# TRI-ML/sdflabel

Hardware: AMD Instinct MI355X
Metric: rendered rays/sec (fwd+bwd) (higher is better)
Workload: dtype f32; 1 GPU; BASELINE configs[1]: one 256x256 crop(s) per GPU, DeepSDF 8x512 on a 40^3 grid, fwd+bwd to yaw/trans/latent, decoder re-evaluated every step; crops_per_gpu=1, rays_per_crop=65536, grid_points=64000, surfels=2751, front_facing=763, parallelism=crop-parallel x1

## Files before the change

sdflabel_amd/csrc/mlp.hip:

```cpp
#include "mlp_kernel.h"
#include <cmath>
#include <stdlib.h>
#include <string.h>
#include <vector>


#define SDFR_DEVICE_CHECK(d, what)                                                                                                          \
    do {                                                                                                                                    \
        int cur_ = -1;                                                                                                                      \
        SDFR_HIP_CHECK(hipGetDevice(&cur_));                                                                                                \
        SDFR_REQUIRE(cur_ == (d)->device, "%s: the decoder's weights live on device %d but the current device (the launch stream's) is %d: " \
                     "create one decoder handle per device", what, (d)->device, cur_);                                                      \
    } while (0)

extern "C" int sdfr_decoder_create(sdfr_decoder** out, int n_lin, const int* in_dim, const int* out_dim,
                                   const int* inj_n, const int* inj_off, const float* const* h_W,
                                   const float* const* h_b, const float* const* h_ln_w, const float* const* h_ln_b, int n_inputs,
                                   int use_tanh, int device) {
    SDFR_REQUIRE(out && in_dim && out_dim && inj_n && inj_off && h_W && h_b, "sdfr_decoder_create: NULL argument");
    SDFR_REQUIRE(n_lin >= 2 && n_lin <= SDFR_MAX_LAYERS, "sdfr_decoder_create: n_lin=%d outside [2,%d]", n_lin, SDFR_MAX_LAYERS);
    SDFR_REQUIRE(out_dim[n_lin - 1] == 1, "sdfr_decoder_create: last layer must have out_dim 1 (got %d)", out_dim[n_lin - 1]);
    SDFR_REQUIRE(in_dim[0] == n_inputs && inj_n[0] == 0, "sdfr_decoder_create: layer 0 must consume exactly the input row");
    int width = 0;
    for (int l = 0; l < n_lin; ++l) {
// ... 36 lines not shown
    for (int l = 0; l < n_lin - 1; ++l) {
        const MlpLayer& L = P.L[l];
        const float* W = h_W[l];
        for (int r = 0; r < L.out_dim; ++r)
            for (int k = 0; k < L.in_dim; ++k) {
                const float w = W[(size_t)r * L.in_dim + k];
                Wf[((size_t)L.off_f + (size_t)(k / 4) * HP + r) * 4 + (k % 4)] = w;
                const _Float16 wh = (_Float16)w;
                const int prev_out = l > 0 ? P.L[l - 1].out_dim : 0;
                const int kh = (kinj && l > 0 && L.inj_n > 0 && k >= prev_out) ? HP + L.inj_off + (k - prev_out) : k;
                Wh[((size_t)L.off_h + (size_t)(kh / 8) * HP + r) * 8 + (kh % 8)] = wh;
                const size_t es = ((size_t)L.off_s + ((size_t)(k / 8) * HP + r) * 2) * 8 + (k % 8);
                Ws[es] = wh;
                Ws[es + 8] = (_Float16)((w - (float)wh) * 2048.f);
                Wb[((size_t)L.off_b + (size_t)(r / 4) * HP + k) * 4 + (r % 4)] = w;
                Wbh[((size_t)L.off_bh + (size_t)(r / 8) * HP + k) * 8 + (r % 8)] = wh;
            }
        for (int r = 0; r < L.out_dim; ++r) bias[(size_t)l * HP + r] = h_b[l][r];
    }
    std::vector<float> Wk;
    bool finite = true;
    if (HP == 512 && !d->has_ln) {
        Wk.assign((size_t)off_f * 4, 0.f);
        for (int l = 0; l < n_lin - 1; ++l) {
            const MlpLayer& L = P.L[l];
            for (int r = 0; r < L.out_dim; ++r)
                for (int k = 0; k < L.in_dim; ++k) {
                    const float w = h_W[l][(size_t)r * L.in_dim + k];
                    finite = finite && std::isfinite(w);
                    Wk[(size_t)L.off_f * 4 + (size_t)k * HP + sdfr_wk_row(r)] = w;
                }
        }
    }
    for (int k = 0; k < in_dim[n_lin - 1]; ++k) wl[k] = h_W[n_lin - 1][k];
    P.b_last = h_b[n_lin - 1][0];

    SDFR_HIP_CHECK(hipMalloc(&d->d_Wf, Wf.size() * sizeof(float)));
    SDFR_HIP_CHECK(hipMalloc(&d->d_Wb, Wb.size() * sizeof(float)));
    if (d->has_ln) {
        std::vector<float> lg((size_t)(n_lin - 1) * HP, 0.f), lb((size_t)(n_lin - 1) * HP, 0.f);
        for (int l = 0; l < n_lin - 1; ++l)
            if (P.L[l].ln)
                for (int r = 0; r < P.L[l].out_dim; ++r) { lg[(size_t)l * HP + r] = h_ln_w[l][r]; lb[(size_t)l * HP + r] = h_ln_b[l][r]; }
        SDFR_HIP_CHECK(hipMalloc(&d->d_lng, lg.size() * sizeof(float)));
        SDFR_HIP_CHECK(hipMalloc(&d->d_lnb, lb.size() * sizeof(float)));
        SDFR_HIP_CHECK(hipMemcpy(d->d_lng, lg.data(), lg.size() * sizeof(float), hipMemcpyHostToDevice));
        SDFR_HIP_CHECK(hipMemcpy(d->d_lnb, lb.data(), lb.size() * sizeof(float), hipMemcpyHostToDevice));
        P.ln_gamma = d->d_lng; P.ln_beta = d->d_lnb;
    }
    SDFR_HIP_CHECK(hipMalloc(&d->d_Wh, Wh.size() * sizeof(_Float16)));
    SDFR_HIP_CHECK(hipMemcpy(d->d_Wh, Wh.data(), Wh.size() * sizeof(_Float16), hipMemcpyHostToDevice));
    SDFR_HIP_CHECK(hipMalloc(&d->d_Wbh, Wbh.size() * sizeof(_Float16)));
    SDFR_HIP_CHECK(hipMemcpy(d->d_Wbh, Wbh.data(), Wbh.size() * sizeof(_Float16), hipMemcpyHostToDevice));
    SDFR_HIP_CHECK(hipMalloc(&d->d_Ws, Ws.size() * sizeof(_Float16)));
    SDFR_HIP_CHECK(hipMemcpy(d->d_Ws, Ws.data(), Ws.size() * sizeof(_Float16), hipMemcpyHostToDevice));
    SDFR_HIP_CHECK(hipMalloc(&d->d_bias, bias.size() * sizeof(float)));
    SDFR_HIP_CHECK(hipMalloc(&d->d_wlast, wl.size() * sizeof(float)));
    SDFR_HIP_CHECK(hipMemcpy(d->d_Wf, Wf.data(), Wf.size() * sizeof(float), hipMemcpyHostToDevice));
    SDFR_HIP_CHECK(hipMemcpy(d->d_Wb, Wb.data(), Wb.size() * sizeof(float), hipMemcpyHostToDevice));
    SDFR_HIP_CHECK(hipMemcpy(d->d_bias, bias.data(), bias.size() * sizeof(float), hipMemcpyHostToDevice));
    SDFR_HIP_CHECK(hipMemcpy(d->d_wlast, wl.data(), wl.size() * sizeof(float), hipMemcpyHostToDevice));
    if (!Wk.empty()) {
        SDFR_HIP_CHECK(hipMalloc(&d->d_Wk, Wk.size() * sizeof(float)));
        SDFR_HIP_CHECK(hipMemcpy(d->d_Wk, Wk.data(), Wk.size() * sizeof(float), hipMemcpyHostToDevice));
        P.Wk = d->d_Wk;
        P.kcompact = finite ? 1 : 0;
    }
    P.Wf = d->d_Wf; P.Wb = d->d_Wb; P.Wh = d->d_Wh; P.Ws = d->d_Ws; P.Wbh = d->d_Wbh; P.bias = d->d_bias; P.w_last = d->d_wlast; P.fwd_np = 2;
    *out = d;
    return SDFR_OK;
}

static unsigned long long* g_trace = nullptr;
extern "C" int sdfr_debug_set_trace(void* device_buffer) { g_trace = (unsigned long long*)device_buffer; return SDFR_OK; }

extern "C" int sdfr_decoder_destroy(sdfr_decoder* d) {
    if (!d) return SDFR_OK;
    void* bufs[] = {d->d_Wf, d->d_Wb, d->d_Wk, d->d_Wh, d->d_Ws, d->d_Wbh, d->d_bias, d->d_wlast, d->d_lng, d->d_lnb, d->ln_ws};
    for (void* b : bufs) (void)hipFree(b);
    delete d;
    return SDFR_OK;
}

extern "C" int64_t sdfr_decoder_macs(const sdfr_decoder* d) { return d ? d->macs : 0; }

static void mask_geometry(int HP, int* ft, int* nt) {
    if (HP == 128) { *ft = 1; *nt = 256; }
    else if (HP == 256) { *ft = 2; *nt = 256; }
    else { *ft = 2; *nt = 512; }
}

extern "C" int64_t sdfr_decoder_mask_words(const sdfr_decoder* d, int64_t n) {
    if (!d || n <= 0) return 0;
    int ft, nt;
    mask_geometry(d->HP, &ft, &nt);
    return ((n + 127) / 128) * 2 * (int64_t)(d->n_lin - 1) * ft * nt;
}

extern "C" int sdfr_mlp_forward(const sdfr_decoder* d, const float* inputs, int64_t n, float* sdf, uint32_t* mask_ws, void* stream) {
    SDFR_REQUIRE(d && inputs && sdf, "sdfr_mlp_forward: NULL argument");
    SDFR_DEVICE_CHECK(d, "sdfr_mlp_forward");
    SDFR_REQUIRE(n >= 0 && n < (int64_t)1 << 31, "sdfr_mlp_forward: n=%lld out of range", (long long)n);
    if (n == 0) return SDFR_OK;
    MlpParams P = d->proto;
    P.inputs = inputs; P.n = n; P.sdf = sdf; P.maskbuf = mask_ws; P.trace = g_trace;
    const int grid = sdfr_cdiv(n, 64);
    if (d->has_ln) sdfr_launch_ln(P, d->HP, false, grid, 1, (hipStream_t)stream);
    else if (d->HP == 512) sdfr_launch_fwd_f32_512(P, n, mask_ws != nullptr, (hipStream_t)stream);
    else sdfr_launch_small(P, d->HP, mask_ws ? 1 : 0, grid, 1, (hipStream_t)stream);
    SDFR_LAUNCH_CHECK();
    return SDFR_OK;
// ... 257 lines not shown
```

sdflabel_amd/csrc/mlp_jac.hip:

```cpp
#include "mlp_kernel.h"
#ifndef SDFR_JAC_MS
#define SDFR_JAC_MS 32
#define SDFR_JAC_FT 4
#define SDFR_JAC_NP 1
#define SDFR_JAC_NW 4
#define SDFR_JAC_PF 2
#endif
#ifndef SDFR_JAC_SMALL_FT
#define SDFR_JAC_SMALL_FT 8
#define SDFR_JAC_SMALL_NW 4
#define SDFR_JAC_SMALL_PF 4
#endif
#ifndef SDFR_JAC_SWITCH_ROWS
#define SDFR_JAC_SWITCH_ROWS 8
#endif
void sdfr_launch_jac_f32_512_recompute32(const MlpParams& P, int cap, int B, hipStream_t s) {
    hipLaunchKernelGGL((sdfr_mlp_kernel<float, 32, 4, 1, 4, 2, 2>), dim3(sdfr_cdiv(cap, 32), B), dim3(256), 0, s, P);
}

#include <stdlib.h>
static int jac_pool_crops() {
    static const int v = [] { const char* e = getenv("SDFR_JAC_POOL_CROPS"); return e ? atoi(e) : 12; }();
    return v;
}
void sdfr_launch_jac_f32_512(const MlpParams& P, int cap, int B, bool from_masks, hipStream_t s) {
    static_assert(SDFR_JAC_MS * SDFR_JAC_FT * SDFR_JAC_NW == 512 && 16 * SDFR_JAC_SMALL_FT * SDFR_JAC_SMALL_NW == 512, "padded width 512 = MS * FT * NW");
    if (!from_masks) {
        hipLaunchKernelGGL((sdfr_mlp_kernel<float, 16, 8, 1, 4, 4, 2>), dim3(sdfr_cdiv(cap, 16), B), dim3(256), 0, s, P);
    } else if (B >= jac_pool_crops() && B <= 64 && P.n_crops == B) {
        const int64_t tiles = (int64_t)sdfr_cdiv(cap, SDFR_JAC_MS * SDFR_JAC_NP) * B;
        hipLaunchKernelGGL((sdfr_mlp_kernel<float, SDFR_JAC_MS, SDFR_JAC_FT, SDFR_JAC_NP, SDFR_JAC_NW, SDFR_JAC_PF, 3, 0, false, 2>),
                           dim3((unsigned)(tiles < 512 ? tiles : 512)), dim3(64 * SDFR_JAC_NW), 0, s, P);
    } else if (B >= SDFR_JAC_SWITCH_ROWS) {
        hipLaunchKernelGGL((sdfr_mlp_kernel<float, SDFR_JAC_MS, SDFR_JAC_FT, SDFR_JAC_NP, SDFR_JAC_NW, SDFR_JAC_PF, 3>),
                           dim3(sdfr_cdiv(cap, SDFR_JAC_MS * SDFR_JAC_NP), B), dim3(64 * SDFR_JAC_NW), 0, s, P);
    } else {
        hipLaunchKernelGGL((sdfr_mlp_kernel<float, 16, SDFR_JAC_SMALL_FT, 1, SDFR_JAC_SMALL_NW, SDFR_JAC_SMALL_PF, 3>), dim3(sdfr_cdiv(cap, 16), B),
                           dim3(64 * SDFR_JAC_SMALL_NW), 0, s, P);
    }
}

void sdfr_launch_fwd_f32_512_tile16(const MlpParams& P, int64_t n, hipStream_t s) {
    hipLaunchKernelGGL((sdfr_mlp_kernel<float, 16, SDFR_JAC_SMALL_FT, 1, SDFR_JAC_SMALL_NW, SDFR_JAC_SMALL_PF, 0>), dim3(sdfr_cdiv(n, 16)),
                       dim3(64 * SDFR_JAC_SMALL_NW), 0, s, P);
}

void sdfr_launch_tail_f32_512(const MlpParams& P, int64_t n_rays, int spec_k, hipStream_t s) {
    const dim3 grid(sdfr_cdiv(n_rays, P.t_rt));
    if (spec_k > 1)
        hipLaunchKernelGGL((sdfr_mlp_kernel<float, 16, SDFR_JAC_SMALL_FT, 4, SDFR_JAC_SMALL_NW, 2, 4>), grid, dim3(64 * SDFR_JAC_SMALL_NW), 0, s, P);
    else
        hipLaunchKernelGGL((sdfr_mlp_kernel<float, 16, SDFR_JAC_SMALL_FT, 1, SDFR_JAC_SMALL_NW, SDFR_JAC_SMALL_PF, 4>), grid, dim3(64 * SDFR_JAC_SMALL_NW), 0,
                           s, P);
}
```

sdflabel_amd/csrc/mlp_kernel.h:

```cpp
#pragma once
#include "sdfr_common.h"
#include "kc_slots.h"
#include <math.h>
#include <type_traits>

typedef float f32x16 __attribute__((ext_vector_type(16)));
typedef float f32x4 __attribute__((ext_vector_type(4)));
typedef _Float16 h16;
typedef h16 h16x8 __attribute__((ext_vector_type(8)));
typedef h16 h16x4 __attribute__((ext_vector_type(4)));

struct MlpLayer {
    int in_dim, out_dim;
    int inj_n, inj_off;
    int kp_f, kp_b, kp_h;
    int off_f, off_b, off_h;
    int kp_bh, off_bh;
    int kp_s, off_s;
    int ln;
};

struct MlpParams {
    const float4* Wf;
    const float4* Wb;
    const void* Wh;
    const void* Wbh;
    const void* Ws;
    const float* Wk;
    int kcompact;
    int kinj;
    int fwd_np;
    const float* bias;
    const float* ln_gamma;
    const float* ln_beta;
    float4* ln_ws;
// ... 18 lines not shown
    int64_t skip_rows;
    const int32_t* crop_cnt;
    int64_t crop_rows;
    const int32_t* gather_idx;
    int64_t gather_rows;
    int n_crops;
    const int32_t* n_dev;
    int n_dev_lo, n_dev_hi;
    unsigned long long* trace;
    float* t_rows;
    int t_rt;
    const float* t_latn;
    const int32_t* t_pix;
    const float4* t_lam;
    int t_step0;
    int t_nlv;
    int t_lv_from[SDFR_TRACE_LEVELS], t_lv_k[SDFR_TRACE_LEVELS];
    float t_qmax;
    int32_t* t_tile_ctr;
    int t_stage;
    int32_t* t_next_cnt;
    int32_t* t_next_pix;
    float4* t_next_lam;
    const float* t_far;
    const float* t_pose;
    const float* t_Kinv;
    float* t_hit_lam;
    float* t_hit_sdf;
    int t_W, t_H, t_steps;
    const int32_t* t_wh; int t_PS;
    float t_eps, t_sigma;
    unsigned long long* t_evals;
    int32_t* t_unresolved;
};

struct sdfr_decoder {
    int device;
    int n_lin, n_inputs, use_tanh, HP;
    float4* d_Wf;
    float4* d_Wb;
    float* d_Wk;
    void* d_Wh;
    void* d_Ws;
    void* d_Wbh;
    float* d_lng;
    float* d_lnb;
    int has_ln;
    mutable float4* ln_ws;
    mutable size_t ln_ws_bytes;
    float* d_bias;
    float* d_wlast;
    int64_t macs;
    MlpParams proto;
};

__device__ __forceinline__ float f4c(const float4& v, int i) { return i == 0 ? v.x : (i == 1 ? v.y : (i == 2 ? v.z : v.w)); }

template <typename ET, int MS> struct Mma;
template <> struct Mma<float, 32> {
    typedef f32x16 acc_t; typedef float4 vec_t;
    static constexpr int KV = 4, NSTEP = 4;
    static __device__ __forceinline__ acc_t step(const vec_t& a, const vec_t& b, acc_t c, int ks) {
        return __builtin_amdgcn_mfma_f32_32x32x2f32(f4c(a, ks), f4c(b, ks), c, 0, 0, 0);
    }
};
template <> struct Mma<float, 16> {
    typedef f32x4 acc_t; typedef float4 vec_t;
    static constexpr int KV = 4, NSTEP = 4;
    static __device__ __forceinline__ acc_t step(const vec_t& a, const vec_t& b, acc_t c, int ks) {
        return __builtin_amdgcn_mfma_f32_16x16x4f32(f4c(a, ks), f4c(b, ks), c, 0, 0, 0);
    }
};
template <> struct Mma<h16, 32> {
    typedef f32x16 acc_t; typedef h16x8 vec_t;
// ... 1 lines not shown
    static __device__ __forceinline__ acc_t step(const vec_t& a, const vec_t& b, acc_t c, int) {
#ifdef SDFR_ABL_NOMFMA
        c[0] += (float)a[0] * (float)b[0];
        return c;
#else
        return __builtin_amdgcn_mfma_f32_32x32x16_f16(a, b, c, 0, 0, 0);
#endif
    }
};
template <> struct Mma<h16, 16> {
    typedef f32x4 acc_t; typedef h16x8 vec_t;
    static constexpr int KV = 8, NSTEP = 1;
    static __device__ __forceinline__ acc_t step(const vec_t& a, const vec_t& b, acc_t c, int) {
        return __builtin_amdgcn_mfma_f32_16x16x32_f16(a, b, c, 0, 0, 0);
    }
};
__device__ __forceinline__ void store4(float* dst, const float* v) { *reinterpret_cast<float4*>(dst) = make_float4(v[0], v[1], v[2], v[3]); }
__device__ __forceinline__ void store4(h16* dst, const float* v) {
    h16x4 t; t[0] = (h16)v[0]; t[1] = (h16)v[1]; t[2] = (h16)v[2]; t[3] = (h16)v[3];
    *reinterpret_cast<h16x4*>(dst) = t;
}

__device__ __forceinline__ int64_t sdfr_mask_dword(int64_t r, int l, int n_layers, int HP32, int j) {
    return (((r >> 7) * n_layers + l) * 128 + (r & 127)) * HP32 + (j >> 5);
}
__host__ __device__ __forceinline__ int sdfr_wk_row(int r) { return (r & ~63) | ((r & 31) << 1) | ((r >> 5) & 1); }
__device__ __forceinline__ int sdfr_mask_shift(int j) { return ((j >> 2) & 1) * 16 + ((j & 31) >> 3) * 4 + (j & 3); }

#ifndef SDFR_MLP_WPE
#define SDFR_MLP_WPE 1
#endif
template <typename ET, int MS, int FT, int NP, int NW, int MODE, bool LN, int XF> constexpr bool sdfr_mlp_kc2() {
    return sizeof(ET) == 4 && MS == 32 && FT == 2 && NP == 1 && NW == 8 && (MODE == 0 || MODE == 1) && !LN && (XF & ~4) == 0;
}
template <typename ET, int MS, int FT, int NP, int NW, int PF, int MODE, int PFB_ = 0, bool LN = false, int XF = 0>
__global__ __launch_bounds__(64 * NW, (sdfr_mlp_kc2<ET, MS, FT, NP, NW, MODE, LN, XF>() ? 4 : SDFR_MLP_WPE)) void sdfr_mlp_kernel(const MlpParams P) {
    typedef Mma<ET, MS> M;
    typedef typename M::acc_t acc_t;
    typedef typename M::vec_t vec_t;
    constexpr bool HALF = sizeof(ET) == 2;
    constexpr bool JAC = MODE == 2 || MODE == 3;
    constexpr bool TAIL = MODE == 4;
    constexpr bool SAVE = MODE == 1;
    constexpr bool LMASK = MODE == 2;
    constexpr bool GMASK = MODE == 3;
    constexpr bool GATHER = (XF & 1) != 0;
    constexpr bool PERSIST = (XF & 2) != 0;
    constexpr bool ORDER = (XF & 4) != 0;
    static_assert(!ORDER || (XF == 4 && (MODE == 0 || MODE == 1) && sizeof(ET) == 4 && MS == 32 && FT == 2), "ORDER: the exact-f32 grid forward alone");
    static_assert(XF == 0 || (MODE == 0 || MODE == 1) || (MODE == 3 && XF == 2), "GATHER is a forward feature; PERSIST: forward modes and the mask-fed Jacobian");
    constexpr bool JPOOL = JAC && PERSIST;
    static_assert(!SAVE || MS == 32, "mask layout assumes 32x32 forward tiles");
    static_assert(!SAVE || (FT * NP) % 2 == 0, "mask words: FT*NP*16 bits per thread and layer must fill whole words");
    static_assert(!HALF || !JAC || MODE == 3, "with half operands only the mask-fed Jacobian exists (MODE 3)");
    static_assert(!LN || (!HALF && MODE != 1 && MODE != 3 && MODE != 4), "LayerNorm decoders: float32 forward (MODE 0) and recomputing Jacobian (MODE 2)");
    static_assert(!TAIL || (NP * MS <= 64 && (NP * MS) % 16 == 0), "tail march: the tile's rows (t_rt rays x K samples) live in wave 0");
    constexpr int KV = M::KV;
    constexpr int NLG = 64 / MS;
    constexpr int RG = MS / (4 * NLG);
    constexpr int KT = KV * NLG;
    constexpr int NT = 64 * NW;
    constexpr int PT = MS * NP;
    constexpr int HP = MS * FT * NW;
    constexpr int KG = HP / KV;
    constexpr int FT32 = HP / (32 * NW);
    constexpr int MW = (FT * NP * RG * 4 + 31) / 32;
    constexpr int MASK_WORDS = LMASK ? (SDFR_MAX_LAYERS * MW * NT) : 1;
    constexpr int LN_F4 = LN ? (NW * PT + SDFR_MAX_LAYERS * PT + 3) / 4 : 0;
    constexpr int KGX = KG + ((HALF && !JAC) ? 4 : 0);
#ifndef SDFR_ACT_DBUF
#define SDFR_ACT_DBUF 1
#endif
    constexpr bool DBUF = SDFR_ACT_DBUF && HALF && !JAC && !LN && !SAVE && (2 * KGX * PT * 16 <= 144 * 1024);
    constexpr int ACT4 = (DBUF ? 2 : 1) * KGX * PT;
    constexpr bool MLDS = GMASK && HALF && MS == 16 && HP == 512;
    static_assert(!MLDS || (FT == 4 && NW == 8), "MLDS: a wave owns 64 features = two mask dwords of a row");
    constexpr int MLDS_WORDS = MLDS ? NW * SDFR_MAX_LAYERS * PT * 2 : 0;
    __shared__ float4 lds4[ACT4 + NT / 4 + 32 + (PT + 3) / 4 * 2 + (MASK_WORDS + 3) / 4 + LN_F4 + (MLDS_WORDS + 3) / 4];
    vec_t* act = reinterpret_cast<vec_t*>(lds4);
    ET* act_e = reinterpret_cast<ET*>(lds4);
    vec_t* actw = DBUF ? act + KGX * PT : act;
    ET* actw_e = reinterpret_cast<ET*>(actw);
    float* red = reinterpret_cast<float*>(lds4 + ACT4);
    int* rows = reinterpret_cast<int*>(lds4 + ACT4 + NT / 4);
    float* gy = reinterpret_cast<float*>(lds4 + ACT4 + NT / 4 + 32);
    int* slots = reinterpret_cast<int*>(lds4 + ACT4 + NT / 4 + 32 + (PT + 3) / 4);
    uint32_t* masks = reinterpret_cast<uint32_t*>(lds4 + ACT4 + NT / 4 + 32 + (PT + 3) / 4 * 2);
    float* lnred = reinterpret_cast<float*>(lds4 + ACT4 + NT / 4 + 32 + (PT + 3) / 4 * 2 + (MASK_WORDS + 3) / 4);
    float* lnrstd = lnred + NW * PT;
    uint32_t* mlds = reinterpret_cast<uint32_t*>(lds4 + ACT4 + NT / 4 + 32 + (PT + 3) / 4 * 2 + (MASK_WORDS + 3) / 4 + LN_F4);
    __shared__ float jinj[MLDS ? PT * 8 : 1];
    __shared__ int jpfx[JPOOL ? 66 : 1];
    constexpr bool KC2 = sdfr_mlp_kc2<ET, MS, FT, NP, NW, MODE, LN, XF>();
    constexpr bool KC = !HALF && MS == 32 && FT == 2 && (NP == 2 || NP == 1) && NW == 8 && (MODE == 0 || MODE == 1) && !LN && (XF & ~4) == 0;
    __shared__ int4 kc_list4[KC ? HP / 4 : 1];
    __shared__ int4 kc_cnt4[KC ? NW / 4 : 1];
    int* kc_cnt = reinterpret_cast<int*>(kc_cnt4);
    constexpr bool KM = KC && NP == 2;
    static_assert(!KC || (KT == 8 && KV == 4 && NW == 8), "kc_slots.h: k tiles of 8, vectors of 4, 8 waves");
    static_assert(!KC2 || (KC && sizeof(lds4) + sizeof(jinj) + sizeof(jpfx) + sizeof(kc_list4) + sizeof(kc_cnt4) <= 80 * 1024),
                  "KC2: two workgroups per CU, at most 80 KiB of LDS each");

    const int tid = threadIdx.x;
    const int wave = __builtin_amdgcn_readfirstlane(tid >> 6);
    const int lane = tid & 63;
    const int lp = lane % MS;
    const int lg = lane / MS;
    const int NI = P.n_inputs;

#ifdef SDFR_MLP_TRACE
#define SDFR_STAMP(l, i)                                                                                                   \
    do {                                                                                                                   \
        if (P.trace && blockIdx.x == 0 && blockIdx.y == 0 && lane == 0 && wave < 8)                                        \
            P.trace[(wave * SDFR_MAX_LAYERS + (l)) * 5 + (i)] = __builtin_amdgcn_s_memtime();                              \
    } while (0)
#else
#define SDFR_STAMP(l, i) do { } while (0)
#endif
    SDFR_STAMP(8, 0);
    int* tile_slot = reinterpret_cast<int*>(gy) + 1;
    int p_iter = 0, p_live = 0;
    bool p_compact = false;
    if constexpr (PERSIST) {
        if (P.crop_cnt && P.n_crops <= PT) {
            if (tid == 0) {
                int acc_ = 0;
                for (int c = 0; c < P.n_crops; ++c) {
                    const int64_t cc = min((int64_t)P.crop_cnt[c], P.crop_rows);
                    acc_ += (int)((cc + PT - 1) / PT);
                    slots[c] = acc_;
                }
                tile_slot[1] = acc_;
// ... 493 lines not shown
        ko[0] = klp[0];
        load_a(ko[0], a[0]);
        load_b(0, b[0]);
        ko[1] = klp[min(1, last) * NLG];
        for (int t = 0; t < nkt; t += 2) {
            load_a(ko[1], a[1]);
            load_b(min(t + 1, last), b[1]);
            ko[0] = klp[min(t + 2, last) * NLG];
            __builtin_amdgcn_sched_barrier(0);
            mma(a[0], b[0]);
            __builtin_amdgcn_sched_barrier(0);
            load_a(ko[0], a[0]);
            load_b(min(t + 2, last), b[0]);
            ko[1] = klp[min(t + 3, last) * NLG];
            __builtin_amdgcn_sched_barrier(0);
            mma(a[1], b[1]);
            __builtin_amdgcn_sched_barrier(0);
        }
    };
    auto gemm_kc = [&](auto Wl, int nk, int rows_active) {
        int nact = (rows_active - fbase + MS - 1) / MS;
        nact = nact < 0 ? 0 : (nact > FT ? FT : nact);
        nact = __builtin_amdgcn_readfirstlane(nact);
        if (!KM || nact != FT || nk < KT) {
#pragma unroll
            for (int f = 0; f < FT; ++f)
#pragma unroll
                for (int p = 0; p < NP; ++p)
#pragma unroll
                    for (int r = 0; r < RG * 4; ++r) acc[f][p][r] = 0.f;
        }
        if (nact == FT) gemm_kc_body(Wl, nk, FT, std::true_type{});
        else if (nact > 0) gemm_kc_body(Wl, nk, nact, std::false_type{});
    };
    auto feat0 = [&](int f, int rg) { return fbase + f * MS + rg * (4 * NLG) + 4 * lg; };
    const vec_t* Wfwd = reinterpret_cast<const vec_t*>(HALF ? (const void*)P.Wh : (const void*)P.Wf);

    auto point_sums = [&](float* v) {
#pragma unroll
        for (int p = 0; p < NP; ++p) {
            float x = v[p];
            for (int o = MS; o < 64; o <<= 1) x += __shfl_xor(x, o, 64);
            if (lg == 0) lnred[wave * PT + p * MS + lp] = x;
        }
        __syncthreads();
#pragma unroll
        for (int p = 0; p < NP; ++p) {
            float t = 0.f;
#pragma unroll
            for (int w = 0; w < NW; ++w) t += lnred[w * PT + p * MS + lp];
            v[p] = t;
        }
        __syncthreads();
    };
    const int64_t wg_lin = (int64_t)blockIdx.y * gridDim.x + blockIdx.x;
    auto ln_forward = [&](int l, int n_out) {
        const float* bias = P.bias + l * HP;
        const float* gam = P.ln_gamma + l * HP;
        const float* bet = P.ln_beta + l * HP;
        float s1[NP], mu[NP], rs[NP];
#pragma unroll
        for (int p = 0; p < NP; ++p) s1[p] = 0.f;
#pragma unroll
        for (int f = 0; f < FT; ++f)
#pragma unroll
            for (int r = 0; r < RG * 4; ++r) {
// ... 434 lines not shown
        if (t_act && t_left > 0) *t_more = 1;
        __syncthreads();
        if (*t_more == 0) break;
        ++t_pass;
        tail_rows(pass_k(P.t_step0 + t_pass), false);
        __syncthreads();
        build_operand();
        __syncthreads();
    }
    } while (TAIL);
    if constexpr (TAIL) {
        if (tid < 64) {
            const unsigned long long left_over = __ballot(t_act && tid < RT);
            const bool hand_over = P.t_next_cnt && (P.t_stage < P.t_steps);
            int base = 0;
            if (tid == 0) {
                if (P.t_evals) atomicAdd(P.t_evals, t_ev);
                if (left_over && !hand_over && P.t_unresolved) atomicAdd(P.t_unresolved, (int)__popcll(left_over));
                if (left_over && hand_over) base = atomicAdd(P.t_next_cnt, (int)__popcll(left_over));
            }
            if (hand_over && left_over) {
                base = __shfl(base, 0, 64);
                if (t_act && tid < RT) {
                    const int at = base + (int)__popcll(left_over & ((1ull << tid) - 1ull));
                    P.t_next_pix[at] = t_gp;
                    P.t_next_lam[at] = t_st;
                }
            }
        }
        if (!P.t_tile_ctr) return;
        continue;
    }
    if constexpr (JAC) {
    __syncthreads();
    SDFR_STAMP(8, 2);

    auto mask_addr = [&](int j, int r, int l, int& shift) -> int64_t {
        shift = sdfr_mask_shift(j);
        return sdfr_mask_dword(r, l - 1, P.n_mfma, HP / 32, j);
    };
    auto fetch_masks = [&](int l, uint32_t* raw) {
#pragma unroll
        for (int p = 0; p < NP; ++p) {
            const int r = rows[p * MS + lp];
#pragma unroll
            for (int f = 0; f < FT; ++f)
#pragma unroll
                for (int rg = 0; rg < RG; ++rg) {
                    int shift;
                    raw[(p * FT + f) * RG + rg] = P.maskbuf[mask_addr(feat0(f, rg), r, l, shift)];
                }
        }
    };
    auto store_in_grad = [&](int l, const uint32_t* raw, auto&& value) {
        const MlpLayer L = P.L[l];
        const int prev_out = P.L[l - 1].out_dim;
        const int inj_hi = prev_out + L.inj_n;
        if constexpr (MLDS) {
            const uint2* mst = reinterpret_cast<const uint2*>(mlds) + ((int64_t)wave * SDFR_MAX_LAYERS + (l - 1)) * PT;
            const int msh = (lg & 1) * 16 + (lg >> 1) * 4;
            uint32_t mk[NP][2];
#pragma unroll
            for (int p = 0; p < NP; ++p) {
                const uint2 m2 = mst[p * MS + lp];
                mk[p][0] = m2.x >> msh; mk[p][1] = m2.y >> msh;
            }
// ... 95 lines not shown
                        const int j0 = feat0(f, rg);
#pragma unroll
                        for (int p = 0; p < NP; ++p) {
                            const float4 xh = xh4[(j0 >> 2) * PT + p * MS + lp];
#pragma unroll
                            for (int i = 0; i < 4; ++i) {
                                const int k = j0 + i;
                                const float gh = (k < prev_out) ? acc[f][p][rg * 4 + i] * gam[k] : 0.f;
                                acc[f][p][rg * 4 + i] = gh;
                                s1[p] += gh;
                                s2[p] += gh * f4c(xh, i);
                            }
                        }
                    }
                point_sums(s1);
                point_sums(s2);
#pragma unroll
                for (int f = 0; f < FT; ++f)
#pragma unroll
                    for (int rg = 0; rg < RG; ++rg) {
                        const int j0 = feat0(f, rg);
#pragma unroll
                        for (int p = 0; p < NP; ++p) {
                            const float4 xh = xh4[(j0 >> 2) * PT + p * MS + lp];
                            const float rs = lnrstd[(l - 1) * PT + p * MS + lp];
                            const float m1 = s1[p] / (float)prev_out, m2 = s2[p] / (float)prev_out;
#pragma unroll
                            for (int i = 0; i < 4; ++i)
                                acc[f][p][rg * 4 + i] = (j0 + i < prev_out) ? rs * (acc[f][p][rg * 4 + i] - m1 - f4c(xh, i) * m2) : 0.f;
                        }
                    }
            }
        }
#pragma unroll
        for (int f = 0; f < FT; ++f)
#pragma unroll
            for (int rg = 0; rg < RG; ++rg) {
                const int j0 = feat0(f, rg);
#pragma unroll
                for (int p = 0; p < NP; ++p) {
                    float v[4];
#pragma unroll
                    for (int i = 0; i < 4; ++i) v[i] = acc[f][p][rg * 4 + i];
                    store4(act_e + ((j0 / KV) * PT + p * MS + lp) * KV + (j0 % KV), v);
                }
            }
    };

    uint32_t raw[NP * FT * RG];
    if (GMASK && !MLDS) fetch_masks(P.n_mfma, raw);
    SDFR_STAMP(8, 3);
    if constexpr (MLDS) {
        if (P.n_mfma >= 1 && !(P.n_mfma - 1 == 0 && P.L[0].in_dim <= 8))
            preload_a(reinterpret_cast<const vec_t*>(P.Wbh) + P.L[P.n_mfma - 1].off_bh);
        float4 wl[FT];
        float gyp[NP];
#pragma unroll
        for (int f = 0; f < FT; ++f) wl[f] = *reinterpret_cast<const float4*>(P.w_last + feat0(f, 0));
#pragma unroll
        for (int p = 0; p < NP; ++p) gyp[p] = gy[p * MS + lp];
        store_in_grad(P.n_mfma, raw, [&](int f, int p, int, int i, int, int) { return f4c(wl[f], i) * gyp[p]; });
    } else
    store_in_grad(P.n_mfma, raw, [&](int, int, int, int, int k, int pt) { return P.w_last[k] * gy[pt]; });
    __syncthreads();
    SDFR_STAMP(8, 4);
    for (int l = P.n_mfma - 1; l >= 0; --l) {
        const MlpLayer L = P.L[l];
        if constexpr (MLDS) {
          if (l == 0 && L.in_dim <= 8) {
            constexpr int TPW = (HP / KT) / NW;
            const vec_t* Wl = reinterpret_cast<const vec_t*>(P.Wbh) + L.off_bh;
            const int nkt = L.kp_bh / KT;
            acc_t a0[NP];
            vec_t av[TPW], bv[TPW][NP];
            SDFR_STAMP(9, 0);
#pragma unroll
            for (int u = 0; u < TPW; ++u) {
                const int t = wave * TPW + u;
#pragma unroll
                for (int i = 0; i < KV; ++i) av[u][i] = (ET)0;
                if (t < nkt) av[u] = Wl[(int64_t)(t * NLG + lg) * HP + lp];
#pragma unroll
                for (int p = 0; p < NP; ++p) bv[u][p] = act[(t * NLG + lg) * PT + p * MS + lp];
// ... 53 lines not shown
                        const cf4p W0c = (cf4p)(uintptr_t)W0;
                        const f32x4 va = W0c[j];
                        f32x4 vb = {0.f, 0.f, 0.f, 0.f};
                        if (L.kp_f > 4) vb = W0c[HP + j];
                        wa = make_float4(va[0], va[1], va[2], va[3]);
                        wb = make_float4(vb[0], vb[1], vb[2], vb[3]);
                    } else {
                        wa = W0[j];
                        wb = (L.kp_f > 4) ? W0[HP + j] : make_float4(0.f, 0.f, 0.f, 0.f);
                    }
                    s8[q][0] = fmaf(wa.x, g, s8[q][0]); s8[q][1] = fmaf(wa.y, g, s8[q][1]); s8[q][2] = fmaf(wa.z, g, s8[q][2]); s8[q][3] = fmaf(wa.w, g, s8[q][3]);
                    s8[q][4] = fmaf(wb.x, g, s8[q][4]); s8[q][5] = fmaf(wb.y, g, s8[q][5]); s8[q][6] = fmaf(wb.z, g, s8[q][6]); s8[q][7] = fmaf(wb.w, g, s8[q][7]);
                }
            }
            SDFR_STAMP(9, 1);
            __syncthreads();
            float* scr = reinterpret_cast<float*>(lds4);
#pragma unroll
            for (int q = 0; q < PPT; ++q)
#pragma unroll
                for (int k = 0; k < 8; ++k) scr[((t0 * PPT + q) * 8 + k) * PT + pt] = s8[q][k];
            __syncthreads();
            for (int e = tid; e < 8 * PT; e += NT) {
                const int k = e / PT, q = e % PT;
                float t = 0.f;
                for (int r = 0; r < PARTS; ++r) t += scr[(r * 8 + k) * PT + q];
                if (k < NI && k < L.in_dim && slots[q] >= 0) atomicAdd(P.J + (int64_t)slots[q] * NI + k, t);
            }
            SDFR_STAMP(9, 2);
            break;
        }
        SDFR_STAMP(l, 0);
        if (GMASK && !MLDS && l > 0) fetch_masks(l, raw);
        gemm(reinterpret_cast<const vec_t*>(HALF ? (const void*)P.Wbh : (const void*)P.Wb) + (HALF ? L.off_bh : L.off_b), HALF ? L.kp_bh : L.kp_b,
             L.in_dim);
        SDFR_STAMP(l, 1);
        __syncthreads();
        SDFR_STAMP(l, 2);
        if (l > 0) {
            if constexpr (MLDS) {
                if (!(l - 1 == 0 && P.L[0].in_dim <= 8)) preload_a(reinterpret_cast<const vec_t*>(P.Wbh) + P.L[l - 1].off_bh);
            }
            store_in_grad(l, raw, [&](int f, int p, int rg, int i, int, int) { return acc[f][p][rg * 4 + i]; });
            SDFR_STAMP(l, 3);
            __syncthreads();
            SDFR_STAMP(l, 4);
            } else {
#pragma unroll
            for (int f = 0; f < FT; ++f)
#pragma unroll
                for (int rg = 0; rg < RG; ++rg) {
                    const int j0 = feat0(f, rg);
                    if (j0 >= NI) continue;
#pragma unroll
                    for (int p = 0; p < NP; ++p) {
                        const int pt = p * MS + lp;
                        if (slots[pt] < 0) continue;
#pragma unroll
                        for (int i = 0; i < 4; ++i)
                            if (j0 + i < NI) atomicAdd(P.J + (int64_t)slots[pt] * NI + j0 + i, acc[f][p][rg * 4 + i]);
                    }
                }
        }
    }
    }
    } while (TAIL || PERSIST);
}


// ... 26 lines not shown
```

Before: 53.26 million rays/s.

## Compact inactive ReLU features in Jacobian backward GEMM via mask-driven k-lists

Adds a compacted backward path for the small-tile Jacobian kernel. Wave-level DPP votes on the ReLU masks build a per-block list of active input features. Gradients are stored densely and the GEMM iterates only over those k tiles, using a pre-permuted weight copy (Wkj) and a 4-deep register ring for weight loads. The aim is to skip MFMA work and weight traffic for features zeroed by ReLU. The cost is extra vote and scatter logic, an additional weight buffer, and padding overhead when few features are inactive.

```diff
diff --git a/sdflabel_amd/csrc/kcj_slots.h b/sdflabel_amd/csrc/kcj_slots.h
--- /dev/null
+++ b/sdflabel_amd/csrc/kcj_slots.h
@@ -0,0 +1,43 @@
+#pragma once
+#include <stdint.h>
+#if defined(__HIPCC__) || defined(__CUDACC__)
+#define SDFR_KCJ_HD __host__ __device__ __forceinline__
+#else
+#define SDFR_KCJ_HD inline
+#endif
+
+constexpr int SDFR_KCJ_PT = 16;
+constexpr int SDFR_KCJ_KT = 16;
+constexpr int SDFR_KCJ_RING = 4;
+
+SDFR_KCJ_HD int sdfr_kcj_popc(uint32_t x) { return __builtin_popcount(x); }
+SDFR_KCJ_HD int sdfr_kcj_count(uint32_t w0, uint32_t w1, uint32_t w2, uint32_t w3) {
+    return sdfr_kcj_popc(w0) + sdfr_kcj_popc(w1) + sdfr_kcj_popc(w2) + sdfr_kcj_popc(w3);
+}
+SDFR_KCJ_HD int sdfr_kcj_rank(uint32_t w0, uint32_t w1, uint32_t w2, uint32_t w3, int q, int g) {
+    const uint32_t below = (uint32_t)((1ull << q) - 1ull);
+    int r = sdfr_kcj_popc(w0 & below) + sdfr_kcj_popc(w1 & below) + sdfr_kcj_popc(w2 & below) + sdfr_kcj_popc(w3 & below);
+    if (g > 0) r += (int)((w0 >> q) & 1u);
+    if (g > 1) r += (int)((w1 >> q) & 1u);
+    if (g > 2) r += (int)((w2 >> q) & 1u);
+    return r;
+}
+SDFR_KCJ_HD int sdfr_kcj_feature(int q, int g) { return (q >> 2) * 16 + 4 * g + (q & 3); }
+SDFR_KCJ_HD int sdfr_kcj_vec(int pos) { return (pos >> 4) * 4 + (pos & 3); }
+SDFR_KCJ_HD int sdfr_kcj_comp(int pos) { return (pos & 15) >> 2; }
+SDFR_KCJ_HD int sdfr_kcj_elem(int pos, int point) { return (sdfr_kcj_vec(pos) * SDFR_KCJ_PT + point) * 4 + sdfr_kcj_comp(pos); }
+SDFR_KCJ_HD int sdfr_kcj_kidx(int pos) { return sdfr_kcj_vec(pos) * 4 + sdfr_kcj_comp(pos); }
+SDFR_KCJ_HD int sdfr_kcj_padded(int tot) {
+    const int trip = SDFR_KCJ_KT * SDFR_KCJ_RING;
+    const int p = (tot + trip - 1) / trip * trip;
+    return p < trip ? trip : p;
+}
+SDFR_KCJ_HD int sdfr_kcj_pad_pos(int tot, int e) { return tot + e / SDFR_KCJ_PT; }
+SDFR_KCJ_HD int sdfr_kcj_pad_point(int e) { return e % SDFR_KCJ_PT; }
+
+SDFR_KCJ_HD int sdfr_kcj_col(int j) { return (j & ~127) | ((j & 15) << 3) | ((j >> 4) & 7); }
+
+SDFR_KCJ_HD int sdfr_kcj_ring_clamp(int tile, int nkt) { return tile < nkt ? tile : nkt - 1; }
+SDFR_KCJ_HD int sdfr_kcj_ring_gather_tile(int t, int nkt) { return sdfr_kcj_ring_clamp(t + SDFR_KCJ_RING - 1, nkt); }
+SDFR_KCJ_HD int sdfr_kcj_ring_klist_tile(int t, int nkt) { return sdfr_kcj_ring_clamp(t + SDFR_KCJ_RING, nkt); }
+SDFR_KCJ_HD int sdfr_kcj_ring_operand_tile(int t, int nkt) { return sdfr_kcj_ring_clamp(t + 1, nkt); }
diff --git a/sdflabel_amd/csrc/mlp.hip b/sdflabel_amd/csrc/mlp.hip
--- a/sdflabel_amd/csrc/mlp.hip
+++ b/sdflabel_amd/csrc/mlp.hip
@@ -92,6 +92,17 @@
                 }
         }
     }
+    std::vector<float> Wkj;
+    bool kcj_ok = HP == 512 && !d->has_ln && n_lin >= 3;
+    for (int l = 1; l < n_lin - 1; ++l) kcj_ok = kcj_ok && in_dim[l] == HP;
+    if (kcj_ok) {
+        Wkj.assign((size_t)off_b * 4, 0.f);
+        for (int l = 0; l < n_lin - 1; ++l) {
+            const MlpLayer& L = P.L[l];
+            for (int r = 0; r < L.out_dim; ++r)
+                for (int k = 0; k < L.in_dim; ++k) Wkj[(size_t)L.off_b * 4 + (size_t)r * HP + sdfr_kcj_col(k)] = h_W[l][(size_t)r * L.in_dim + k];
+        }
+    }
     for (int k = 0; k < in_dim[n_lin - 1]; ++k) wl[k] = h_W[n_lin - 1][k];
     P.b_last = h_b[n_lin - 1][0];
 
@@ -126,6 +137,12 @@
         P.Wk = d->d_Wk;
         P.kcompact = finite ? 1 : 0;
     }
+    if (!Wkj.empty()) {
+        SDFR_HIP_CHECK(hipMalloc(&d->d_Wkj, Wkj.size() * sizeof(float)));
+        SDFR_HIP_CHECK(hipMemcpy(d->d_Wkj, Wkj.data(), Wkj.size() * sizeof(float), hipMemcpyHostToDevice));
+        P.Wkj = d->d_Wkj;
+        P.jcompact = finite ? 1 : 0;
+    }
     P.Wf = d->d_Wf; P.Wb = d->d_Wb; P.Wh = d->d_Wh; P.Ws = d->d_Ws; P.Wbh = d->d_Wbh; P.bias = d->d_bias; P.w_last = d->d_wlast; P.fwd_np = 2;
     *out = d;
     return SDFR_OK;
@@ -136,7 +153,7 @@
 
 extern "C" int sdfr_decoder_destroy(sdfr_decoder* d) {
     if (!d) return SDFR_OK;
-    void* bufs[] = {d->d_Wf, d->d_Wb, d->d_Wk, d->d_Wh, d->d_Ws, d->d_Wbh, d->d_bias, d->d_wlast, d->d_lng, d->d_lnb, d->ln_ws};
+    void* bufs[] = {d->d_Wf, d->d_Wb, d->d_Wk, d->d_Wkj, d->d_Wh, d->d_Ws, d->d_Wbh, d->d_bias, d->d_wlast, d->d_lng, d->d_lnb, d->ln_ws};
     for (void* b : bufs) (void)hipFree(b);
     delete d;
     return SDFR_OK;
diff --git a/sdflabel_amd/csrc/mlp_jac.hip b/sdflabel_amd/csrc/mlp_jac.hip
--- a/sdflabel_amd/csrc/mlp_jac.hip
+++ b/sdflabel_amd/csrc/mlp_jac.hip
@@ -35,8 +35,11 @@
         hipLaunchKernelGGL((sdfr_mlp_kernel<float, SDFR_JAC_MS, SDFR_JAC_FT, SDFR_JAC_NP, SDFR_JAC_NW, SDFR_JAC_PF, 3>),
                            dim3(sdfr_cdiv(cap, SDFR_JAC_MS * SDFR_JAC_NP), B), dim3(64 * SDFR_JAC_NW), 0, s, P);
     } else {
+        MlpParams Q = P;
+        const char* e = getenv("SDFR_JAC_COMPACT");
+        if (e && e[0] == '0') Q.jcompact = 0;
         hipLaunchKernelGGL((sdfr_mlp_kernel<float, 16, SDFR_JAC_SMALL_FT, 1, SDFR_JAC_SMALL_NW, SDFR_JAC_SMALL_PF, 3>), dim3(sdfr_cdiv(cap, 16), B),
-                           dim3(64 * SDFR_JAC_SMALL_NW), 0, s, P);
+                           dim3(64 * SDFR_JAC_SMALL_NW), 0, s, Q);
     }
 }
 
diff --git a/sdflabel_amd/csrc/mlp_kernel.h b/sdflabel_amd/csrc/mlp_kernel.h
--- a/sdflabel_amd/csrc/mlp_kernel.h
+++ b/sdflabel_amd/csrc/mlp_kernel.h
@@ -1,6 +1,7 @@
 #pragma once
 #include "sdfr_common.h"
 #include "kc_slots.h"
+#include "kcj_slots.h"
 #include <math.h>
 #include <type_traits>
 
@@ -85,6 +86,8 @@
     float t_eps, t_sigma;
     unsigned long long* t_evals;
     int32_t* t_unresolved;
+    const float* Wkj;
+    int jcompact;
 };
 
 struct sdfr_decoder {
@@ -93,6 +96,7 @@
     float4* d_Wf;
     float4* d_Wb;
     float* d_Wk;
+    float* d_Wkj;
     void* d_Wh;
     void* d_Ws;
     void* d_Wbh;
@@ -160,6 +164,9 @@
 #endif
 template <typename ET, int MS, int FT, int NP, int NW, int MODE, bool LN, int XF> constexpr bool sdfr_mlp_kc2() {
     return sizeof(ET) == 4 && MS == 32 && FT == 2 && NP == 1 && NW == 8 && (MODE == 0 || MODE == 1) && !LN && (XF & ~4) == 0;
+}
+template <typename ET, int MS, int FT, int NP, int NW, int MODE, bool LN, int XF> constexpr bool sdfr_mlp_kcj() {
+    return sizeof(ET) == 4 && MS == 16 && NP == 1 && NW == 4 && FT == 8 && MODE == 3 && !LN && XF == 0;
 }
 template <typename ET, int MS, int FT, int NP, int NW, int PF, int MODE, int PFB_ = 0, bool LN = false, int XF = 0>
 __global__ __launch_bounds__(64 * NW, (sdfr_mlp_kc2<ET, MS, FT, NP, NW, MODE, LN, XF>() ? 4 : SDFR_MLP_WPE)) void sdfr_mlp_kernel(const MlpParams P) {
@@ -226,6 +233,10 @@
     int* kc_cnt = reinterpret_cast<int*>(kc_cnt4);
     constexpr bool KM = KC && NP == 2;
     static_assert(!KC || (KT == 8 && KV == 4 && NW == 8), "kc_slots.h: k tiles of 8, vectors of 4, 8 waves");
+    constexpr bool KCJ = sdfr_mlp_kcj<ET, MS, FT, NP, NW, MODE, LN, XF>();
+    __shared__ int4 kcj_list4[KCJ ? HP / 4 : 1];
+    __shared__ int4 kcj_cnt4[1];
+    static_assert(!KCJ || (KT == SDFR_KCJ_KT && PT == SDFR_KCJ_PT && KV == 4 && PF == SDFR_KCJ_RING && MW == 1), "kcj_slots.h: 16-row tiles, k tiles of 16, ring of 4");
     static_assert(!KC2 || (KC && sizeof(lds4) + sizeof(jinj) + sizeof(jpfx) + sizeof(kc_list4) + sizeof(kc_cnt4) <= 80 * 1024),
                   "KC2: two workgroups per CU, at most 80 KiB of LDS each");
 
@@ -785,6 +796,51 @@
         }
         if (nact == FT) gemm_kc_body(Wl, nk, FT, std::true_type{});
         else if (nact > 0) gemm_kc_body(Wl, nk, nact, std::false_type{});
+    };
+    auto gemm_kcj = [&](const float* __restrict__ Wl, int nk) {
+        if constexpr (KCJ) {
+        const int nkt = nk / KT;
+        const uint32_t wlane4 = (uint32_t)(fbase + 8 * lp) * 4u;
+        const vec_t* bptr = act + lg * PT + lp;
+        const int4* klp = kcj_list4 + lg;
+        float4 a[SDFR_KCJ_RING][4][2], b[2];
+        auto load_a = [&](const int4& k, float4 (*aa)[2]) {
+#pragma unroll
+            for (int ks = 0; ks < 4; ++ks) {
+                const int kk = ks == 0 ? k.x : ks == 1 ? k.y : ks == 2 ? k.z : k.w;
+                const float4* wp = reinterpret_cast<const float4*>(reinterpret_cast<const char*>(Wl) + (uint32_t)((uint32_t)kk * 4u + wlane4));
+                aa[ks][0] = wp[0];
+                aa[ks][1] = wp[1];
+            }
+        };
+        int4 ko = klp[0];
+#pragma unroll
+        for (int u = 0; u < SDFR_KCJ_RING - 1; ++u) {
+            load_a(ko, a[u]);
+            ko = klp[sdfr_kcj_ring_clamp(u + 1, nkt) * NLG];
+        }
+        b[0] = bptr[0];
+#pragma unroll
+        for (int f = 0; f < FT; ++f)
+#pragma unroll
+            for (int r = 0; r < 4; ++r) acc[f][0][r] = 0.f;
+        __builtin_amdgcn_sched_barrier(0);
+        for (int t = 0; t < nkt; t += SDFR_KCJ_RING) {
+#pragma unroll
+            for (int u = 0; u < SDFR_KCJ_RING; ++u) {
+                load_a(ko, a[(u + SDFR_KCJ_RING - 1) % SDFR_KCJ_RING]);
+                b[(u + 1) % 2] = bptr[sdfr_kcj_ring_operand_tile(t + u, nkt) * (NLG * PT)];
+                ko = klp[sdfr_kcj_ring_klist_tile(t + u, nkt) * NLG];
+                __builtin_amdgcn_sched_barrier(0);
+#pragma unroll
+                for (int ks = 0; ks < 4; ++ks)
+#pragma unroll
+                    for (int f = 0; f < FT; ++f)
+                        acc[f][0] = __builtin_amdgcn_mfma_f32_16x16x4f32(f4c(a[u][ks][f >> 2], f & 3), f4c(b[u % 2], ks), acc[f][0], 0, 0, 0);
+                __builtin_amdgcn_sched_barrier(0);
+            }
+        }
+        }
     };
     auto feat0 = [&](int f, int rg) { return fbase + f * MS + rg * (4 * NLG) + 4 * lg; };
     const vec_t* Wfwd = reinterpret_cast<const vec_t*>(HALF ? (const void*)P.Wh : (const void*)P.Wf);
@@ -1285,6 +1341,42 @@
         continue;
     }
     if constexpr (JAC) {
+    uint32_t raw[NP * FT * RG];
+    const bool kcj_on = KCJ && P.jcompact && P.Wkj;
+    uint32_t kcj_w[4] = {0u, 0u, 0u, 0u};
+    int kcj_n = 0;
+    auto kcj_vote = [&](int l, const uint32_t* raw) {
+        const int prev_out = P.L[l - 1].out_dim;
+        uint32_t m = 0u;
+#pragma unroll
+        for (int f = 0; f < FT; ++f) m |= ((raw[f] >> sdfr_mask_shift(fbase + f * MS + 4 * lg)) & 0xFu) << (4 * f);
+        if (__builtin_amdgcn_readfirstlane((int)(fbase + MS * FT > prev_out)) != 0) {
+            uint32_t keep = 0u;
+#pragma unroll
+            for (int f = 0; f < FT; ++f) {
+                const int nv = min(max(prev_out - (fbase + f * MS + 4 * lg), 0), 4);
+                keep |= ((1u << nv) - 1u) << (4 * f);
+            }
+            m &= keep;
+        }
+        int x = (int)m;
+        x |= __builtin_amdgcn_update_dpp(0, x, 0xB1, 0xf, 0xf, false);
+        x |= __builtin_amdgcn_update_dpp(0, x, 0x4E, 0xf, 0xf, false);
+        x |= __builtin_amdgcn_update_dpp(0, x, 0x124, 0xf, 0xf, false);
+        x |= __builtin_amdgcn_update_dpp(0, x, 0x128, 0xf, 0xf, false);
+#pragma unroll
+        for (int g = 0; g < 4; ++g) kcj_w[g] = (uint32_t)__builtin_amdgcn_readlane(x, 16 * g);
+        if (lane == 0) reinterpret_cast<int*>(kcj_cnt4)[wave] = sdfr_kcj_count(kcj_w[0], kcj_w[1], kcj_w[2], kcj_w[3]);
+    };
+    const bool kcj_top = kcj_on && P.n_mfma >= 2;
+    if constexpr (KCJ) {
+        if (kcj_top) {
+            const int r = rows[lp];
+#pragma unroll
+            for (int f = 0; f < FT; ++f) raw[f] = P.maskbuf[sdfr_mask_dword(r, P.n_mfma - 1, P.n_mfma, HP / 32, fbase + f * MS + 4 * lg)];
+            kcj_vote(P.n_mfma, raw);
+        }
+    }
     __syncthreads();
     SDFR_STAMP(8, 2);
 
@@ -1446,6 +1538,45 @@
                     }
             }
         }
+        if constexpr (KCJ) {
+            if (kcj_on && l >= 2) {
+                const int4 c4 = kcj_cnt4[0];
+                const int c[4] = {c4.x, c4.y, c4.z, c4.w};
+                int off = 0, tot = 0;
+#pragma unroll
+                for (int w = 0; w < 4; ++w) {
+                    off += w < wave ? c[w] : 0;
+                    tot += c[w];
+                }
+                off = __builtin_amdgcn_readfirstlane(off);
+                tot = __builtin_amdgcn_readfirstlane(tot);
+                const uint32_t mine = lg == 0 ? kcj_w[0] : lg == 1 ? kcj_w[1] : lg == 2 ? kcj_w[2] : kcj_w[3];
+                int n = off;
+#pragma unroll
+                for (int q = 0; q < 32; ++q) {
+                    const int b0 = (int)((kcj_w[0] >> q) & 1u), b1 = (int)((kcj_w[1] >> q) & 1u), b2 = (int)((kcj_w[2] >> q) & 1u),
+                              b3 = (int)((kcj_w[3] >> q) & 1u);
+                    const int front = ((b0 << 2) | ((b0 + b1) << 4) | ((b0 + b1 + b2) << 6)) >> (2 * lg) & 3;
+                    if ((mine >> q) & 1u) act_e[sdfr_kcj_elem(n + front, lp)] = acc[q >> 2][0][q & 3];
+                    n += b0 + b1 + b2 + b3;
+                }
+#pragma unroll
+                for (int h = 0; h < 2; ++h) {
+                    const int q = lp + 16 * h;
+                    if ((mine >> q) & 1u)
+                        reinterpret_cast<int*>(kcj_list4)[sdfr_kcj_kidx(off + sdfr_kcj_rank(kcj_w[0], kcj_w[1], kcj_w[2], kcj_w[3], q, lg))] =
+                            (fbase + sdfr_kcj_feature(q, lg)) * HP;
+                }
+                const int padded = sdfr_kcj_padded(tot);
+                for (int e = tid; e < (padded - tot) * PT; e += NT) {
+                    const int pos = sdfr_kcj_pad_pos(tot, e);
+                    act_e[sdfr_kcj_elem(pos, sdfr_kcj_pad_point(e))] = 0.f;
+                    if (sdfr_kcj_pad_point(e) == 0) reinterpret_cast<int*>(kcj_list4)[sdfr_kcj_kidx(pos)] = 0;
+                }
+                kcj_n = padded;
+                return;
+            }
+        }
 #pragma unroll
         for (int f = 0; f < FT; ++f)
 #pragma unroll
@@ -1461,8 +1592,7 @@
             }
     };
 
-    uint32_t raw[NP * FT * RG];
-    if (GMASK && !MLDS) fetch_masks(P.n_mfma, raw);
+    if (GMASK && !MLDS && !kcj_top) fetch_masks(P.n_mfma, raw);
     SDFR_STAMP(8, 3);
     if constexpr (MLDS) {
         if (P.n_mfma >= 1 && !(P.n_mfma - 1 == 0 && P.L[0].in_dim <= 8))
@@ -1582,9 +1712,18 @@
         }
         SDFR_STAMP(l, 0);
         if (GMASK && !MLDS && l > 0) fetch_masks(l, raw);
+        bool kcj_l = false;
+        if constexpr (KCJ) kcj_l = kcj_on && l >= 1;
+        if constexpr (KCJ) {
+            if (kcj_l) gemm_kcj(P.Wkj + (int64_t)L.off_b * 4, kcj_n);
+        }
+        if (!kcj_l)
         gemm(reinterpret_cast<const vec_t*>(HALF ? (const void*)P.Wbh : (const void*)P.Wb) + (HALF ? L.off_bh : L.off_b), HALF ? L.kp_bh : L.kp_b,
              L.in_dim);
         SDFR_STAMP(l, 1);
+        if constexpr (KCJ) {
+            if (kcj_on && l >= 2) kcj_vote(l, raw);
+        }
         __syncthreads();
         SDFR_STAMP(l, 2);
         if (l > 0) {
```

Result: faster. 54.00 million rays/s, median of 6 (+1.4%).
